# Pixie8888/R3DFSSeg

Measured on AMD Instinct MI355X. Metric: episodes/sec S3DIS 2-way 5-shot 2048-pt (MPTI+attention, train step: forward+backward+grad all-reduce+Adam), higher is better.
Workload: dtype f32 (index-free GEMMs -- self-attention, 1x1 convolutions, weight gradients, the EdgeConv backward's edge GEMMs -- as bf16x3 split products on the bf16 MFMA with fp32 accumulate; every index-deciding result: fp32)

## Files before the change

### include/r3d.h

```cpp
#ifndef R3D_H
#define R3D_H
#include <stdint.h>

#ifdef __cplusplus
extern "C" {
#endif

const char* r3d_last_error_string(void);
int r3d_abi_version(void);
int r3d_debug_poison_lds(unsigned pattern, unsigned* sink , void* stream);
int r3d_debug_set_cg_spmv_lds_min_blocks(int min_blocks);
int r3d_set_matrix_arith(int mode);
int r3d_get_matrix_arith(void);
int r3d_debug_set_gemm_bx3(int mask);

int r3d_cm_to_pm(const float* in , int B, int C, int N, float* out , long ld, void* stream);
int r3d_pm_to_cm(const float* in , long ld, int B, int C, int N, float* out , void* stream);
long r3d_cm_pitch(int N);
int r3d_copy_cols(const float* src, long ld_src, float* dst, long ld_dst, long M, int C, void* stream);

long r3d_knn_norm_ws_words(int B, int N);
int r3d_knn_topk(const float* x, long ldx, const float* x_cm, int B, int N, int C, int k, int mode,
                 const int32_t* n_valid_dev, float* norm_ws, float* cm_ws, int32_t* idx_out, float* score_out,
                 int32_t* status, void* stream);
// ... 46 lines not shown
                        int max_iter, float tol, float* Z, int32_t* ws, long ws_words, int32_t* stats_out, void* stream);

int r3d_label_propagate_batched(int n_ep, const float* nodes, long ldn, int D, const int32_t* nbr, int kp1, const float* Y,
                                const int32_t* n_dev, const int32_t* n_proto_dev, long desc_stride, int n_cap, float sigma,
                                float alpha, int max_iter, float tol, float* Z, int32_t* ws, long ws_words, long ws_stride,
                                int32_t* stats_out, long stats_stride, void* stream);
long r3d_graph_weights_verify_words(int n_cap, int kp1);
int r3d_graph_weights_verify(int n_ep, const float* nodes, long ldn, int D, const int32_t* n_dev, long desc_stride, int n_cap,
                             int kp1, float sigma, int32_t* ws, long ws_words, long ws_stride, float* scratch,
                             int32_t* mismatch_out, void* stream);

int r3d_label_propagate_solve_batched(int n_ep, const float* Y, const int32_t* n_dev, long desc_stride, int n_cap, int kp1,
                                      float alpha, int max_iter, float tol, float* Z, int32_t* ws, long ws_words,
                                      long ws_stride, int32_t* stats_out, long stats_stride, void* stream);

int r3d_graph_set_lp_budget(void* graph, void* graph_exec, int budget, int* n_cg);

int r3d_query_logits_ce_batched(int n_ep, const float* Z, long z_ep_rows, const int32_t* n_proto_dev, long desc_stride, int n_q,
                                int N, int n_classes, const int64_t* labels, float* logits, float* loss_out, int32_t* pred_out,
                                void* stream);

int r3d_pointwise_conv_acc(const float* X, long ldx, const float* W, long M, int K, int Co, const float* scale,
                           const float* shift, int act, float* Out, long ldo, void* stream);
long r3d_pointwise_conv_stats_ws_words(long M, int Co);
int r3d_pointwise_conv_stats(const float* X, long ldx, const float* W, long M, int K, int Co, float* Out, long ldo,
                             float* sums_out , float* ws, void* stream);
int r3d_pointwise_conv_stats_seg(const float* X, long ldx, const float* W, long M, int K, int Co, float* Out, long ldo,
                                 long rows_a, long rows_b, float* sums_out, float* ws, void* stream);
long r3d_colstats_seg_ws_words(long M, int C, long rows_a, long rows_b);
int r3d_colstats_seg(const float* X, long ldx, const float* DY, long lddy, long M, int C, long rows_a, long rows_b, int mode,
                     const float* scale, const float* shift, const float* mean, const float* invstd, long bn_stride, int act,
                     float* sums_out , float* ws, void* stream);
int r3d_bn_fold_seg(const float* sums , int n_seg, double count_a, double count_b, int C, const float* gamma,
                    const float* beta, float eps, float momentum, float* running_mean , float* running_var ,
                    float* mean, float* invstd, float* scale, float* shift, long bn_stride, float* rec ,
                    const int32_t* rec_index_dev , long rec_stride, void* stream);
int r3d_affine_act_seg(const float* Z, long ldz, long M, int C, long rows_a, long rows_b, const float* scale, const float* shift,
                       long bn_stride, int act, float* Y, long ldy, void* stream);
int r3d_bn_bwd_apply_seg(const float* Z, long ldz, const float* DY, long lddy, long M, int C, long rows_a, long rows_b,
                         const float* scale, const float* shift, const float* mean, const float* invstd, long bn_stride, int act,
                         const float* sums , double count_a, double count_b, float* DZ, long lddz, void* stream);
int r3d_bn_running_update(const float* rec, int n_records, long rec_stride, int C, float momentum,
                          const float* bias , float* running_mean,
                          float* running_var, void* stream);
long r3d_gemm_tn_ws_words(long M, int Ca, int Cb);
int r3d_gemm_tn(const float* A, long lda, const float* B, long ldb, long M, int Ca, int Cb, float alpha, float* out,
                int accumulate, float* ws, void* stream);
int r3d_add_cols(const float* src, long ld_src, float* dst, long ld_dst, long M, int C, void* stream);

long r3d_edgeconv_train_ws_words(int B, int N);
int r3d_edge_stats1(const float* PQ, const int32_t* idx, int B, int N, int K, int clouds_a, int clouds_b,
                    float* sums_out , float* esum , float* ws,
                    void* stream);
int r3d_edgeconv_train_fwd_minmax(const float* PQ, const int32_t* idx, const float* s1, const float* t1, long bn_stride,
                                  const float* W2, int B, int N, int K, int clouds_a, int clouds_b, float* zmax, float* zmin,
                                  int32_t* argmax, int32_t* argmin, float* sums_out , float* ws, void* stream);
int r3d_edge_select(float* zmax , const float* zmin, int32_t* argmax ,
                    const int32_t* argmin, const float* s2, const float* t2, long bn_stride, long M, long rows_a, long rows_b,
                    float* out, long ldo, void* stream);
long r3d_edge_reverse_ws_words(int B, int N, int K);
int r3d_edge_reverse(const int32_t* idx, int B, int N, int K, int32_t* rev_ws, long ws_words, void* stream);
int r3d_edgeconv_bwd(const float* PQ, const int32_t* idx, const float* s1, const float* t1, const float* mean1,
                     const float* invstd1, const float* W2, const float* s2, const float* t2, const float* mean2,
                     const float* invstd2, long bn_stride, const float* bn2_sums, const float* dout, long lddo,
                     const int32_t* argmax, const float* zwin , const float* esum , int B, int N, int K,
                     int clouds_a, int clouds_b, float* DY1 , float* BE ,
                     const int32_t* rev_ws , float* dW2, float* bn1_sums, float* dPQ,
                     float* ws, void* stream);

int r3d_ce_grad_batched(int n_ep, const float* Z, const int32_t* n_proto_dev, long desc_stride, int n_cap, int n_query_pts,
                        int n_classes, const int64_t* labels, const float* gscale_dev, float* G, void* stream);
int r3d_label_propagate_bwd_batched(int n_ep, const float* nodes, long ldn, int D, int kp1, const float* Z, const float* G,
                                    const int32_t* n_dev, long desc_stride, int n_cap, float sigma, float alpha, int max_iter,
                                    float tol, float* lam, float* dnodes, long ldd, int32_t* ws, long ws_words, long ws_stride,
                                    int32_t* stats_out, long stats_stride, void* stream);
int r3d_head_prototypes_bwd_batched(int n_ep, const float* dnodes, long ldd, long nodes_ep_rows, int n_way, int k_shot, int N,
                                    int D, int n_query_pts, const int32_t* desc, long desc_stride, const int32_t* assign,
                                    long assign_stride, const int32_t* cluster_count, long ccount_stride, const int32_t* ws,
                                    long ws_stride, float* dsfeat, long lds_, long dsfeat_ep_rows, float* dqfeat, long ldq,
                                    long dqfeat_ep_rows, void* stream);

long r3d_contrast_ws_words(int n_way, int k_shot, int N);
int r3d_contrast_fwd(const float* feat, long ldf, int D, const int32_t* support_y, const int32_t* support_flag, int n_way,
                     int k_shot, int N, const float* W, const float* bias, float temp, float* loss_out, float* ws,
                     long ws_words, void* stream);
int r3d_contrast_bwd(int D, int n_way, int k_shot, int N, const float* gscale_dev, float* dfeat, long ldd, float* dW,
                     float* db, float* ws, void* stream);
int r3d_contrast_fwd_batched(int n_ep, const float* feat, long ldf, long feat_ep_rows, int D, const int32_t* support_y,
                             const int32_t* support_flag, int n_way, int k_shot, int N, const float* W, const float* bias,
                             float temp, float* loss_out, float* ws, long ws_words, long ws_stride, void* stream);
int r3d_contrast_bwd_batched(int n_ep, int D, int n_way, int k_shot, int N, const float* gscale_dev, float* dfeat, long ldd,
                             long dfeat_ep_rows, float* dW, float* db, float* ws, long ws_stride, void* stream);
int r3d_train_metrics_batched(int n_ep, const int32_t* pred, const int64_t* query_y, const int64_t* gt_query_y, int n_query_pts,
                              const float* Z, long z_ep_rows, const int32_t* desc, long desc_stride, const int32_t* proto_ws,
                              long pws_stride, const int32_t* assign, long assign_stride, const int32_t* gt_support_y, int n_way,
                              int k_shot, int N, float* out4 , void* stream);

long r3d_clean_ws_words(int n_way, int k_shot);
int r3d_clean_shot_detect_batched(int n_ep, const float* feat, long ldf, long feat_ep_rows, int D, const float* support_x,
                                  int Cin, const int32_t* support_y, int n_way, int k_shot, int N, int32_t* shot_keep,
                                  float* dbg_cos_sum, int32_t* ws, long ws_stride, void* stream);

int r3d_protonet_head(const float* sfeat, long ldf, const float* qfeat, long ldq, int D, const int32_t* support_y,
                      int n_way, int k_shot, int N, int n_query_pts, int method, float scaler, float* Z, float* ws,
                      void* stream);

long r3d_protonet_head_ws_words(int n_ep, int n_way, int k_shot);
int r3d_protonet_head_batched(int n_ep, const float* sfeat, long ldf, const float* qfeat, long ldq, long feat_ep_rows, int D,
                              const int32_t* support_y, int n_way, int k_shot, int N, int n_query_pts, int method,
                              float scaler, float* Z, float* ws, long ws_words, void* stream);
int r3d_count_correct_batched(int n_ep, const int32_t* pred, const int64_t* labels, long n_pts, int32_t* correct,
                              void* stream);
// ... 22 lines not shown
```

### r3dfsseg_amd/csrc/edgeconv_train.hip

```cpp
#include <stdlib.h>
#include "edge_tile.h"

#define ET_LD 65
#define ET_MAXBLK 1024
#define EC_CHUNK 32

static __device__ __forceinline__ float lrelu(float v) { return v > 0.f ? v : 0.2f * v; }

struct EcGeom {
  int N, cpc;
  __host__ __device__ static EcGeom make(int N) { return EcGeom{N, (N + EC_CHUNK - 1) / EC_CHUNK}; }
  __device__ void range(int chunk, int& cloud, int& p0, int& p1) const {
    cloud = __builtin_amdgcn_readfirstlane(chunk / cpc);
    p0 = __builtin_amdgcn_readfirstlane(cloud * N + (chunk - cloud * cpc) * EC_CHUNK);
    p1 = __builtin_amdgcn_readfirstlane(min(p0 + EC_CHUNK, (cloud + 1) * N));
  }
};
static __device__ __forceinline__ int ec_seg(const r3d_segmap& cs, int cloud) {
  return __builtin_amdgcn_readfirstlane(cs.seg_of_row32(cloud));
}

template <int RT>
__global__ __launch_bounds__(256) void r3d_edge_stats1_kernel(const float* __restrict__ PQ, const int* __restrict__ idx,
                                                              EcGeom gm, int n_chunks, float* __restrict__ part,
// ... 180 lines not shown
#pragma unroll 4
      for (int s = 0; s < 4 * RT; ++s) {
        const int e = 16 * (s >> 2) + 4 * g + (s & 3);
        const float a = G[e * E2_LD + 16 * w + n];
        const float4 b = *(const float4*)(H + e * E2_LD + 4 * n);
        dw[0] = mfma16(a, b.x, dw[0]);
        dw[1] = mfma16(a, b.y, dw[1]);
        dw[2] = mfma16(a, b.z, dw[2]);
        dw[3] = mfma16(a, b.w, dw[3]);
      }
      __syncthreads();
#pragma unroll
      for (int t = 0; t < RT; ++t) {
#pragma unroll
        for (int i = 0; i < 4; ++i) G[(16 * t + 4 * g + i) * E2_LD + c] = acc[t][i];
      }
      __syncthreads();
      {
        float* drow = DY1 + ((pt0 + w) * K) * 64 + lane;
        const float* grow = G + (K * w) * E2_LD + lane;
        float bs = 0.f, es = 0.f;
#pragma unroll
        for (int t = 0; t < K; ++t) {
          const float v = grow[t * E2_LD];
          drow[t * 64] = v;
          bs += v;
          es += eh[t];
          sdye += v * eh[t];
        }
        sdy += bs;
        BE[(pt0 + w) * 128 + lane] = bs;
        BE[(pt0 + w) * 128 + 64 + lane] = es;
      }
    }
    float (*ps)[2][64] = (float (*)[2][64])dsm;
    ps[w][0][lane] = sdy;
    ps[w][1][lane] = sdye;
    __syncthreads();
    if (tid < 128) {
      const int v = tid >> 6, cc = tid & 63;
      part_bn[((long)chunk * 2 + v) * 64 + cc] = ((ps[0][v][cc] + ps[1][v][cc]) + ps[2][v][cc]) + ps[3][v][cc];
    }
    __syncthreads();
  }
  int tid2 = threadIdx.x;
  asm volatile("" : "+v"(tid2));
  const int w2 = tid2 >> 6, n2 = tid2 & 15, g2 = (tid2 >> 4) & 3;
  float* mypart = part_dw + (long)blockIdx.x * 4096;
#pragma unroll
  for (int i = 0; i < 4; ++i)
    *(float4*)(mypart + (16 * w2 + 4 * g2 + i) * 64 + 4 * n2) = float4{dw[0][i], dw[1][i], dw[2][i], dw[3][i]};
}

template <int RT>
__global__ __launch_bounds__(256) void r3d_edgeconv_train_fwd2_kernel(
    const float* __restrict__ PQ, const int* __restrict__ idx, const float* __restrict__ s1, const float* __restrict__ t1,
    long bn_stride, const float* __restrict__ W2, EcGeom gm, r3d_segmap cs , int n_chunks,
    int* __restrict__ argmax_out, float* __restrict__ zmax_out, float* __restrict__ zmin_out, int* __restrict__ argmin_out,
    float* __restrict__ part ) {
  constexpr int K = 4 * RT, R = 16 * RT;
  extern __shared__ __attribute__((aligned(16))) float smem[];
  float* H = smem;
  float* Z = smem + R * E2_LD;
  const int tid = threadIdx.x, lane = tid & 63, w = tid >> 6;
  const int n = lane & 15, g = lane >> 4;
  const int c = 16 * w + n;
  const int N = gm.N;
  float Bz[16];
#pragma unroll
  for (int s = 0; s < 16; ++s) Bz[s] = W2[c * 64 + 16 * g + s];
  for (int item = blockIdx.x; item < n_chunks; item += gridDim.x) {
    const int chunk = r3d_xcd_swizzle(item, n_chunks);
    int cloud, p0, p1;
    gm.range(chunk, cloud, p0, p1);
    const long cloud0 = (long)cloud * N;
    const long bo = (long)ec_seg(cs, cloud) * bn_stride;
    const float sc1 = s1[bo + lane], sh1 = t1[bo + lane];
    float za = 0.f, zb = 0.f;
    for (int pt0_ = p0; pt0_ < p1; pt0_ += E2_PTS) {
      const long pt0 = pt0_;
      {
        const int my_idx = min(max(idx[(pt0 + w) * K + min(lane, K - 1)], 0), N - 1);
        const float q = PQ[(pt0 + w) * 128 + 64 + lane];
        float pv[K];
#pragma unroll
        for (int t = 0; t < K; ++t) pv[t] = PQ[(cloud0 + __builtin_amdgcn_readlane(my_idx, t)) * 128 + lane];
        float* hrow = H + (K * w) * E2_LD + lane;
#pragma unroll
        for (int t = 0; t < K; ++t) hrow[t * E2_LD] = lrelu(sc1 * (pv[t] + q) + sh1);
      }
      __syncthreads();
      f32x4 acc[RT];
      e2_rowgemm<RT>(H, Bz, n, g, acc);
#pragma unroll
      for (int t = 0; t < RT; ++t) {
#pragma unroll
        for (int i = 0; i < 4; ++i) {
          const float z = acc[t][i];
          za += z;
          zb += z * z;
          Z[(16 * t + 4 * g + i) * E2_LD + c] = z;
        }
      }
      __syncthreads();
      {
        const float* zp = Z + (K * w) * E2_LD + lane;
        float zx = zp[0], zn = zx;
        int ax = 0, an = 0;
#pragma unroll
        for (int t = 1; t < K; ++t) {
          const float z = zp[t * E2_LD];
          if (z > zx) { zx = z; ax = t; }
          if (z < zn) { zn = z; an = t; }
        }
        const long o = (pt0 + w) * 64 + lane;
        zmax_out[o] = zx;
        zmin_out[o] = zn;
        argmax_out[o] = ax;
        argmin_out[o] = an;
      }
    }
    za += __shfl_xor(za, 16); zb += __shfl_xor(zb, 16);
    za += __shfl_xor(za, 32); zb += __shfl_xor(zb, 32);
    if (g == 0) {
      part[((long)chunk * 2 + 0) * 64 + c] = za;
      part[((long)chunk * 2 + 1) * 64 + c] = zb;
    }
  }
}

#define RV_RANGE 256
#define RV_CAP 12288
__global__ __launch_bounds__(1024) void r3d_edge_reverse_kernel(const int* __restrict__ idx, int N, int K, int n_clouds,
                                                                int* __restrict__ rev_ptr, int* __restrict__ rev) {
  __shared__ int cnt[RV_RANGE];
  __shared__ int off[RV_RANGE + 1];
  __shared__ int cur[RV_RANGE];
  __shared__ int buf[RV_CAP];
  __shared__ int wsum[16];
  __shared__ int below_s, b_s;
  const int tid = threadIdx.x, lane = tid & 63, w = tid >> 6;
  const int cloud = blockIdx.y;
  const int r0 = blockIdx.x * RV_RANGE, nr = min(RV_RANGE, N - r0);
  const long E = (long)N * K, gbase = (long)cloud * E;
  const int* lst = idx + gbase;
  if (tid < RV_RANGE) cnt[tid] = 0;
  if (tid == 0) below_s = 0;
  __syncthreads();
  int my_below = 0;
  for (long e0 = tid; e0 < E; e0 += 8 * 1024) {
    int jv[8];
#pragma unroll
    for (int u = 0; u < 8; ++u) jv[u] = lst[min(e0 + 1024 * u, E - 1)];
#pragma unroll
    for (int u = 0; u < 8; ++u) {
      const int j = min(max(jv[u], 0), N - 1) - r0;
      if (e0 + 1024 * u < E) {
        if (j < 0) ++my_below;
        else if (j < nr) atomicAdd(&cnt[j], 1);
      }
    }
  }
#pragma unroll
  for (int o = 32; o > 0; o >>= 1) my_below += __shfl_xor(my_below, o);
  if (lane == 0) atomicAdd(&below_s, my_below);
  __syncthreads();
  if (tid < RV_RANGE) {
    const int v = tid < nr ? cnt[tid] : 0;
    int x = v;
#pragma unroll
    for (int o = 1; o < 64; o <<= 1) {
      const int y = __shfl_up(x, o);
      if (lane >= o) x += y;
    }
    if (lane == 63) wsum[w] = x;
    cur[tid] = x - v;
  }
  __syncthreads();
  if (tid < RV_RANGE) {
    int wb = 0;
    for (int q = 0; q < w; ++q) wb += wsum[q];
// ... 189 lines not shown
    }
  }
}

static int et_check(const char* fn, int B, int N, int K, int clouds_a, int clouds_b) {
  if (B <= 0 || N <= 0 || N % E2_PTS != 0 || K < 4 || K > 32 || K % 4 != 0) {
    r3d_set_error("%s: unsupported shape B=%d N=%d K=%d (N %% 4 == 0, K %% 4 == 0, 4..32)", fn, B, N, K);
    return R3D_ERR_ARG;
  }
  const r3d_segmap cs{clouds_a, clouds_b};
  if (!cs.covers(B)) {
    r3d_set_error("%s: %d clouds are not whole segments of %d + %d clouds", fn, B, clouds_a, clouds_b);
    return R3D_ERR_ARG;
  }
  if ((long)B * N * K >= 0x7fffffffL) {
    r3d_set_error("%s: B*N*K = %ld edges exceed the 31-bit edge ids", fn, (long)B * N * K);
    return R3D_ERR_ARG;
  }
  return 0;
}
static int et_chunks(int B, int N) { return B * EcGeom::make(N).cpc; }
static int et_grid8(int n_chunks, int cap) { return n_chunks <= cap ? n_chunks : (cap >= 8 ? cap & ~7 : cap); }

extern "C" long r3d_edgeconv_train_ws_words(int B, int N) { return (long)ET_MAXBLK * 4096 + (long)et_chunks(B, N) * 128 + 64; }

static void et_reduce_chunks(const float* part, int N, int clouds_a, int clouds_b, int n_seg, float* out, hipStream_t st) {
  const int cpc = EcGeom::make(N).cpc;
  hipLaunchKernelGGL(r3d_part_reduce_kernel, dim3(128 / 64, n_seg), dim3(1024), 0, st, part, clouds_a * cpc, clouds_b * cpc, 128,
                     out, 128L, 128, (float*)nullptr, 0L);
}

extern "C" int r3d_edge_stats1(const float* PQ, const int32_t* idx, int B, int N, int K, int clouds_a, int clouds_b,
                               float* sums_out, float* esum, float* ws, void* stream) {
  R3D_REQUIRE(PQ && idx && sums_out && ws, "r3d_edge_stats1: null pointer");
  int rc = et_check("r3d_edge_stats1", B, N, K, clouds_a, clouds_b);
  if (rc) return rc;
  hipStream_t st = (hipStream_t)stream;
  const EcGeom gm = EcGeom::make(N);
  const int n_chunks = et_chunks(B, N);
  const int grid = et_grid8(n_chunks, 2048);
#define E2_CASE(RT) \
  case RT: hipLaunchKernelGGL(r3d_edge_stats1_kernel<RT>, dim3(grid), dim3(256), 0, st, PQ, idx, gm, n_chunks, ws, esum); break
  switch (K / 4) {
    E2_CASE(1); E2_CASE(2); E2_CASE(3); E2_CASE(4); E2_CASE(5); E2_CASE(6); E2_CASE(7); E2_CASE(8);
  }
#undef E2_CASE
  et_reduce_chunks(ws, N, clouds_a, clouds_b, r3d_segmap{clouds_a, clouds_b}.n_seg(B), sums_out, st);
  R3D_LAUNCH_CHECK("r3d_edge_stats1");
  return R3D_OK;
}

template <int RT>
static int fwd2_launch_rt(int n_chunks, hipStream_t st, const float* PQ, const int32_t* idx, const float* s1, const float* t1,
                          long bn_stride, const float* W2, EcGeom gm, r3d_segmap cs, int32_t* argmax, float* zmax, float* zmin,
                          int32_t* argmin, float* ws) {
  const size_t lds = sizeof(float) * ((size_t)2 * 16 * RT * E2_LD);
  static int resident = 0;
  if (!resident) {
    resident = e2_resident_blocks(r3d_edgeconv_train_fwd2_kernel<RT>, lds, ET_MAXBLK);
    R3D_REQUIRE(resident > 0, "r3d_edgeconv_train_fwd_minmax: cannot reserve %zu B of LDS", lds);
  }
  const int grid = et_grid8(n_chunks, resident);
  hipLaunchKernelGGL(r3d_edgeconv_train_fwd2_kernel<RT>, dim3(grid), dim3(256), lds, st, PQ, idx, s1, t1, bn_stride, W2, gm, cs,
                     n_chunks, argmax, zmax, zmin, argmin, ws);
  return R3D_OK;
}

extern "C" int r3d_edgeconv_train_fwd_minmax(const float* PQ, const int32_t* idx, const float* s1, const float* t1,
                                             long bn_stride, const float* W2, int B, int N, int K, int clouds_a, int clouds_b,
                                             float* zmax, float* zmin, int32_t* argmax, int32_t* argmin, float* sums_out,
                                             float* ws, void* stream) {
  R3D_REQUIRE(PQ && idx && s1 && t1 && W2 && zmax && zmin && argmax && argmin && sums_out && ws,
              "r3d_edgeconv_train_fwd_minmax: null pointer");
  int rc = et_check("r3d_edgeconv_train_fwd_minmax", B, N, K, clouds_a, clouds_b);
  if (rc) return rc;
  hipStream_t st = (hipStream_t)stream;
  const EcGeom gm = EcGeom::make(N);
  const r3d_segmap cs{clouds_a, clouds_b};
  const int n_chunks = et_chunks(B, N);
#define E2_CASE(RT)                                                                                                    \
  case RT:                                                                                                             \
    rc = fwd2_launch_rt<RT>(n_chunks, st, PQ, idx, s1, t1, bn_stride, W2, gm, cs, argmax, zmax, zmin, argmin, ws);      \
    break
  switch (K / 4) {
    E2_CASE(1); E2_CASE(2); E2_CASE(3); E2_CASE(4); E2_CASE(5); E2_CASE(6); E2_CASE(7); E2_CASE(8);
  }
#undef E2_CASE
  if (rc) return rc;
  et_reduce_chunks(ws, N, clouds_a, clouds_b, cs.n_seg(B), sums_out, st);
  R3D_LAUNCH_CHECK("r3d_edgeconv_train_fwd_minmax");
  return R3D_OK;
}

__global__ void r3d_edge_select_kernel(float* __restrict__ zmax, const float* __restrict__ zmin, int* __restrict__ argmax,
                                       const int* __restrict__ argmin, const float* __restrict__ s2,
                                       const float* __restrict__ t2, long bn_stride, r3d_segmap sm , long M,
                                       float* __restrict__ out, long ldo) {
  const long i = (long)blockIdx.x * blockDim.x + threadIdx.x;
  if (i >= M * 64) return;
  const int c = (int)(i & 63);
  const long m = (long)__builtin_amdgcn_readfirstlane((int)(i >> 6));
  const long bo = (long)__builtin_amdgcn_readfirstlane(sm.seg_of_row32((int)m)) * bn_stride + c;
  const float sc = s2[bo];
  const bool up = sc >= 0.f;
  const float z = up ? zmax[i] : zmin[i];
  if (!up) { zmax[i] = z; argmax[i] = argmin[i]; }
  out[m * ldo + c] = lrelu(sc * z + t2[bo]);
}
extern "C" int r3d_edge_select(float* zmax, const float* zmin, int32_t* argmax, const int32_t* argmin, const float* s2,
                               const float* t2, long bn_stride, long M, long rows_a, long rows_b, float* out, long ldo,
                               void* stream) {
  R3D_REQUIRE(zmax && zmin && argmax && argmin && s2 && t2 && out && M > 0 && ldo >= 64, "r3d_edge_select: bad arguments");
  const r3d_segmap sm{rows_a, rows_b};
  R3D_REQUIRE(sm.covers(M), "r3d_edge_select: %ld rows are not whole segments of %ld + %ld rows", M, rows_a, rows_b);
  hipLaunchKernelGGL(r3d_edge_select_kernel, dim3(r3d_cdiv(M * 64, 256)), dim3(256), 0, (hipStream_t)stream, zmax, zmin,
                     argmax, argmin, s2, t2, bn_stride, sm, M, out, ldo);
  R3D_LAUNCH_CHECK("r3d_edge_select");
  return R3D_OK;
}

template <int RT>
static int bwd1_launch_rt(int n_chunks, hipStream_t st, const float* PQ, const int32_t* idx, EcBn bn, const float* W2,
                          const float* bn2_sums, const float* dout, long lddo, const int32_t* argmax, EcGeom gm, r3d_segmap cs,
                          float* DY1, float* BE, float* part_dw, float* part_bn, int* grid_out) {
  const size_t lds = sizeof(float) * ((size_t)2 * 16 * RT * E2_LD + 2 * E2_PTS * 64 + 6 * 64);
  static int resident = 0;
  if (!resident) {
    resident = e2_resident_blocks(r3d_edgeconv_bwd1_kernel<RT>, lds, ET_MAXBLK);
    R3D_REQUIRE(resident > 0, "r3d_edgeconv_bwd: cannot reserve %zu B of LDS", lds);
  }
  const int grid = et_grid8(n_chunks, resident);
  hipLaunchKernelGGL(r3d_edgeconv_bwd1_kernel<RT>, dim3(grid), dim3(256), lds, st, PQ, idx, bn, W2, bn2_sums, dout, lddo, argmax,
                     gm, cs, n_chunks, DY1, BE, part_dw, part_bn);
  *grid_out = grid;
  return R3D_OK;
}

template <int RT>
static int bwd1_bx3_launch_rt(int n_chunks, hipStream_t st, const float* PQ, const int32_t* idx, EcBn bn, const float* W2,
                              const float* bn2_sums, const float* dout, long lddo, const int32_t* argmax, const float* zwin,
                              EcGeom gm, r3d_segmap cs, float* DY1, float* BE, float* part_dw, float* part_bn, int* grid_out) {
  static int resident = 0;
  if (!resident) {
    resident = e2_resident_blocks(r3d_edgeconv_bwd1_bx3_kernel<RT>, EB_LDS_BYTES, ET_MAXBLK / 2);
    R3D_REQUIRE(resident > 0, "r3d_edgeconv_bwd: cannot reserve %d B of LDS", (int)EB_LDS_BYTES);
  }
  const int grid = et_grid8(n_chunks, resident);
  hipLaunchKernelGGL(r3d_edgeconv_bwd1_bx3_kernel<RT>, dim3(grid), dim3(256), EB_LDS_BYTES, st, PQ, idx, bn, W2, bn2_sums, dout,
                     lddo, argmax, zwin, gm, cs, n_chunks, DY1, BE, part_dw, part_bn);
  *grid_out = grid;
  return R3D_OK;
}

extern "C" long r3d_edge_reverse_ws_words(int B, int N, int K) { return (long)B * N + 1 + (long)B * N * K + 16; }
extern "C" int r3d_edge_reverse(const int32_t* idx, int B, int N, int K, int32_t* rev_ws, long ws_words, void* stream) {
  R3D_REQUIRE(idx && rev_ws, "r3d_edge_reverse: null pointer");
  R3D_REQUIRE(B > 0 && B <= 65535 && N > 0 && K > 0 && (long)B * N * K < 0x7fffffffL, "r3d_edge_reverse: bad shape B=%d N=%d K=%d",
              B, N, K);
  R3D_REQUIRE(ws_words >= r3d_edge_reverse_ws_words(B, N, K), "r3d_edge_reverse: workspace of %ld words is shorter than "
              "r3d_edge_reverse_ws_words(%d, %d, %d)", ws_words, B, N, K);
  const size_t ro_lds = sizeof(int) * (size_t)RO_WAVES * N;
  static const bool ro_off = getenv("R3D_EDGE_REVERSE_SORT") != nullptr;
  if (!ro_off && ro_lds <= 144 * 1024 && (long)N * K >= 64 * RO_WAVES) {
    static size_t attr = 0;
    if (ro_lds > attr) {
      R3D_REQUIRE(hipFuncSetAttribute((const void*)r3d_edge_reverse_ordered_kernel, hipFuncAttributeMaxDynamicSharedMemorySize,
                                      (int)ro_lds) == hipSuccess, "r3d_edge_reverse: cannot reserve %zu B of LDS", ro_lds);
      attr = ro_lds;
    }
    hipLaunchKernelGGL(r3d_edge_reverse_ordered_kernel, dim3(B), dim3(64 * RO_WAVES), ro_lds, (hipStream_t)stream, idx, N, K, B,
// ... 61 lines not shown
```

### r3dfsseg_amd/train_ops.py

```python
import contextlib
import ctypes
from collections import namedtuple

import torch

from . import _lib, ops
from .ops import SegLayout, _p, _rows, _st, _timed

BN_EPS, BN_MOM = 1e-5, 0.1
update_running_stats = True


class BNRecorder:

    def __init__(self, max_episodes, device):
        self.max_records = 2 * max_episodes
        self.device = device
        self.tables = {}
        self.index_dev = None

    def slot_for(self, bnmod, bias):
        if bnmod not in self.tables:
            rec = torch.zeros(self.max_records, 2, bnmod.num_features, device=self.device, dtype=torch.float32)
            self.tables[bnmod] = (rec, bias.detach() if bias is not None else None)
# ... 144 lines not shown
    M, ldx = _rows(X)
    C = W2d.shape[0]
    lib = _lib.load()
    seg = _one_segment(M) if seg is None else seg
    assert seg.M == M
    z = torch.empty(M, C, device=X.device, dtype=torch.float32)
    if seg.aligned(64):
        sums = _f(seg.n_seg * 2 * C, X.device).view(seg.n_seg, 2, C)
        ws = _f(lib.r3d_pointwise_conv_stats_ws_words(M, C), X.device)
        with _timed("pointwise_conv"):
            _lib.check(lib.r3d_pointwise_conv_stats_seg(_p(X), ldx, _p(W2d), M, X.shape[1], C, _p(z), C, seg.rows_a, seg.rows_b,
                                                        _p(sums), _p(ws), _st()))
    else:
        ops.pointwise_conv(X, W2d, out=z)
        sums = colstats(z, C, seg, mode=0)
    bn = bn_fold(sums, seg.counts(), bnmod, bias)
    y = affine_act(z, bn, act, seg, out=out)
    return y, (X, W2d, z, bn, act, seg)


def conv_bn_bwd(saved, dY, want_dx=True, dx_acc=None):
    X, W2d, z, bn, act, seg = saved
    C = W2d.shape[0]
    M = z.shape[0]
    sums = colstats(z, C, seg, mode=1, DY=dY, bn=bn, act=act)
    dz = bn_bwd_apply(z, dY, bn, act, sums, seg.counts(), seg)
    dW = gemm_tn(dz, X)
    tot = sums.sum(0) if seg.n_seg > 1 else sums[0]
    dbias = torch.zeros(C, device=z.device, dtype=torch.float32)
    dX = None
    if want_dx:
        Wt = W2d.t().contiguous()
        if dx_acc is not None:
            conv_acc(dz, Wt, dx_acc)
        else:
            dX = ops.pointwise_conv(dz, Wt)
    return dW, tot[1], tot[0], dbias, dX


def edgeconv_train_fwd(inp, idx, ec, B, N, out, seg=None):
    lib = _lib.load()
    dev = inp.device
    seg = SegLayout(1, B, 0, N) if seg is None else seg
    assert seg.B == B and seg.N == N
    W1 = ec.layer[0].weight.reshape(64, -1)
    C = W1.shape[1] // 2
    Wpq = torch.cat((W1[:, :C], W1[:, C:] - W1[:, :C]), 0).contiguous()
    PQ = ops.pointwise_conv(inp, Wpq)
    K = idx.shape[-1]
    ws = _f(lib.r3d_edgeconv_train_ws_words(B, N), dev)
    W2 = ec.layer[3].weight.reshape(64, 64).contiguous()
    M = B * N
    argmax = torch.empty(M, 64, device=dev, dtype=torch.int32)
    argmin = torch.empty(M, 64, device=dev, dtype=torch.int32)
    zmax = torch.empty(M, 64, device=dev, dtype=torch.float32)
    zmin = torch.empty(M, 64, device=dev, dtype=torch.float32)
    idx3 = idx.view(B, N, K)
    sums1 = _f(seg.n_seg * 128, dev).view(seg.n_seg, 2, 64)
    sums2 = _f(seg.n_seg * 128, dev).view(seg.n_seg, 2, 64)
    counts = seg.counts(per_row=K)
    esum = torch.empty(M, 64, device=dev, dtype=torch.float32)
    with _timed("edgeconv"):
        _lib.check(lib.r3d_edge_stats1(_p(PQ), _p(idx3), B, N, K, seg.S, seg.Q, _p(sums1), _p(esum), _p(ws), _st()))
    bn1 = bn_fold(sums1, counts, ec.layer[1])
    sc1, sh1, _, _ = bn1.ptrs()
    with _timed("edgeconv"):
        _lib.check(lib.r3d_edgeconv_train_fwd_minmax(_p(PQ), _p(idx3), sc1, sh1, bn1.stride, _p(W2), B, N, K, seg.S, seg.Q,
                                                     _p(zmax), _p(zmin), _p(argmax), _p(argmin), _p(sums2), _p(ws), _st()))
    bn2 = bn_fold(sums2, counts, ec.layer[4])
    sc2, sh2, _, _ = bn2.ptrs()
    with _timed("edgeconv"):
        _lib.check(lib.r3d_edge_select(_p(zmax), _p(zmin), _p(argmax), _p(argmin), sc2, sh2, bn2.stride, M, seg.rows_a,
                                       seg.rows_b, _p(out), out.stride(0), _st()))
    return (inp, idx3, Wpq, PQ, W2, bn1, bn2, argmax, zmax, C, seg, esum)


def edgeconv_train_bwd(saved, dout, B, N, dx_acc):
    inp, idx3, Wpq, PQ, W2, bn1, bn2, argmax, zmax, C, seg, esum = saved
    lib = _lib.load()
    dev = PQ.device
    K = idx3.shape[-1]
    M = B * N
    dPQ = _f(M * 128, dev).view(M, 128)
    ws = _f(lib.r3d_edgeconv_train_ws_words(B, N), dev)
    rev = torch.empty(lib.r3d_edge_reverse_ws_words(B, N, K), device=dev, dtype=torch.int32)
    with _timed("edgeconv_bwd"):
        _lib.check(lib.r3d_edge_reverse(_p(idx3), B, N, K, _p(rev), rev.numel(), _st()))
    bn2_sums = colstats(zmax, 64, seg, mode=1, DY=dout, bn=bn2, act=ops.ACT_LRELU)
    DY1, BE = _f(M * K * 64, dev), _f(M * 128, dev)
    dW2, bn1_sums = _f(64 * 64, dev), _f(seg.n_seg * 128, dev).view(seg.n_seg, 2, 64)
    s1, t1, m1, i1 = bn1.ptrs()
    s2, t2, m2, i2 = bn2.ptrs()
    with _timed("edgeconv_bwd"):
        _lib.check(lib.r3d_edgeconv_bwd(_p(PQ), _p(idx3), s1, t1, m1, i1, _p(W2), s2, t2, m2, i2, bn1.stride, _p(bn2_sums),
                                        _p(dout), dout.stride(0), _p(argmax), _p(zmax), _p(esum), B, N, K, seg.S, seg.Q, _p(DY1),
                                        _p(BE), _p(rev),
                                        _p(dW2), _p(bn1_sums), _p(dPQ), _p(ws), _st()))
    t1s = bn1_sums.sum(0) if seg.n_seg > 1 else bn1_sums[0]
    t2s = bn2_sums.sum(0) if seg.n_seg > 1 else bn2_sums[0]
    dWpq = gemm_tn(dPQ, inp)
    dW1 = torch.cat((dWpq[:64] - dWpq[64:], dWpq[64:]), 1).reshape(64, 2 * C, 1, 1)
    if dx_acc is not None:
        conv_acc(dPQ, Wpq.t().contiguous(), dx_acc)
    return dW1, t1s[1], t1s[0], dW2.view(64, 64, 1, 1), t2s[1], t2s[0]


EncoderSaved = namedtuple("EncoderSaved", "model seg seed p_drop seed_dev ec mlp base cat level2 qkv lse feat aws")


def encoder_forward(model, x, seed, seg=None):
    enc, base, att = model.encoder, model.base_learner, model.att_learner
    lib = _lib.load()
    B, _, N = x.shape
    M = B * N
    dev = x.device
    if seg is None:
        seg = SegLayout(1, B, 0, N)
    assert seg.B == B and seg.N == N
    x_pm, x_cm = ops.input_layouts(x)
    cat = torch.empty(M, 64 * enc.n_edgeconv, device=dev, dtype=torch.float32)
    inp, ec_saved = x_pm, []
    for l in range(enc.n_edgeconv):
        idx = ops.knn(inp, B, N, enc.k, x_cm=x_cm if l == 0 else None)
        if enc.idx_patch is not None:
            idx = enc.idx_patch(l, idx.view(B, N, enc.k)).view(idx.shape)
        out = cat[:, 64 * l:64 * (l + 1)]
        ec_saved.append(edgeconv_train_fwd(inp, idx, enc.edge_convs[l], B, N, out, seg))
        inp = out
    h, mlp_saved = cat, []
    for jn in range(len(enc.conv.layer_dims)):
        W = enc.conv.layer[3 * jn].weight
        h, sv = conv_bn_fwd(h, W.reshape(W.shape[0], -1).contiguous(), enc.conv.layer[3 * jn + 1], ops.ACT_LRELU, seg=seg)
        mlp_saved.append(sv)
    level2 = h
    feat = torch.empty(M, model.feat_dim, device=dev, dtype=torch.float32)
    od = att.out_channel
    ops.copy_cols(cat[:, :64], feat[:, :64])
    hb, base_saved = level2, []
    for i, seq in enumerate(base.convs):
        last = i == base.num_convs - 1
        W = seq[0].weight
        hb, sv = conv_bn_fwd(hb, W.reshape(W.shape[0], -1).contiguous(), seq[1], ops.ACT_NONE if last else ops.ACT_RELU,
                             bias=seq[0].bias, out=feat[:, 64 + od:] if last else None, seg=seg)
        base_saved.append(sv)
    Wqkv, qscale = att._fold()
    qkv = ops.pointwise_conv(level2, Wqkv, qscale, None, ops.ACT_NONE)
    lse = torch.empty(M, device=dev, dtype=torch.float32)
    p_drop = float(att.dropout.p)
# ... 150 lines not shown
```

Baseline: 384.9.

## Select EdgeConv max/min winner in-register using BN gamma sign, double-buffer gather

The EdgeConv forward kernel now reads the sign of BN2's gamma to decide whether each channel keeps the max or the min over neighbours. It picks that winner directly from the MFMA accumulators with a sign-flip trick and permlane swaps, writing only one value and one index instead of max, min and both argmax/argmin. This drops the Z staging in LDS, one barrier per tile, half the output writes and the separate edge_select kernel, which is replaced by a generic affine_act. The gather of the next tile's neighbour features and indices is software-pipelined through cursors and double-buffered H in LDS. The risks are more register pressure and a dependence on gamma's sign standing in for the folded BN scale's sign, which holds if the folded scale is gamma times a positive inverse std.

Result: no change. 388.5, median of 6 (+1.0%).

```diff
diff --git a/include/r3d.h b/include/r3d.h
--- a/include/r3d.h
+++ b/include/r3d.h
@@ -122,12 +122,9 @@
 int r3d_edge_stats1(const float* PQ, const int32_t* idx, int B, int N, int K, int clouds_a, int clouds_b,
                     float* sums_out , float* esum , float* ws,
                     void* stream);
-int r3d_edgeconv_train_fwd_minmax(const float* PQ, const int32_t* idx, const float* s1, const float* t1, long bn_stride,
-                                  const float* W2, int B, int N, int K, int clouds_a, int clouds_b, float* zmax, float* zmin,
-                                  int32_t* argmax, int32_t* argmin, float* sums_out , float* ws, void* stream);
-int r3d_edge_select(float* zmax , const float* zmin, int32_t* argmax ,
-                    const int32_t* argmin, const float* s2, const float* t2, long bn_stride, long M, long rows_a, long rows_b,
-                    float* out, long ldo, void* stream);
+int r3d_edgeconv_train_fwd_win(const float* PQ, const int32_t* idx, const float* s1, const float* t1, long bn_stride,
+                               const float* W2, const float* gamma2, int B, int N, int K, int clouds_a, int clouds_b,
+                               float* zwin, int32_t* argwin, float* sums_out , float* ws, void* stream);
 long r3d_edge_reverse_ws_words(int B, int N, int K);
 int r3d_edge_reverse(const int32_t* idx, int B, int N, int K, int32_t* rev_ws, long ws_words, void* stream);
 int r3d_edgeconv_bwd(const float* PQ, const int32_t* idx, const float* s1, const float* t1, const float* mean1,
diff --git a/r3dfsseg_amd/csrc/edgeconv_train.hip b/r3dfsseg_amd/csrc/edgeconv_train.hip
--- a/r3dfsseg_amd/csrc/edgeconv_train.hip
+++ b/r3dfsseg_amd/csrc/edgeconv_train.hip
@@ -256,81 +256,149 @@
     *(float4*)(mypart + (16 * w2 + 4 * g2 + i) * 64 + 4 * n2) = float4{dw[0][i], dw[1][i], dw[2][i], dw[3][i]};
 }
 
+struct EcCursor {
+  int item, chunk, cloud, p0, p1, pt0;
+  long bo;
+  __device__ bool valid(int n_chunks) const { return item < n_chunks; }
+  __device__ void open(const EcGeom& gm, const r3d_segmap& cs, long bn_stride, int n_chunks) {
+    if (item < n_chunks) {
+      chunk = r3d_xcd_swizzle(item, n_chunks);
+      gm.range(chunk, cloud, p0, p1);
+      pt0 = p0;
+      bo = (long)ec_seg(cs, cloud) * bn_stride;
+    }
+  }
+  __device__ void next(const EcGeom& gm, const r3d_segmap& cs, long bn_stride, int n_chunks, int stride) {
+    pt0 += E2_PTS;
+    if (pt0 >= p1 && item < n_chunks) {
+      item += stride;
+      open(gm, cs, bn_stride, n_chunks);
+    }
+  }
+};
+
+static __device__ __forceinline__ void ec_better(float& av, int& ap, float bv, int bp) {
+  const bool take = (bv > av) | ((bv == av) & (bp < ap));
+  av = take ? bv : av;
+  ap = take ? bp : ap;
+}
+
 template <int RT>
 __global__ __launch_bounds__(256) void r3d_edgeconv_train_fwd2_kernel(
     const float* __restrict__ PQ, const int* __restrict__ idx, const float* __restrict__ s1, const float* __restrict__ t1,
-    long bn_stride, const float* __restrict__ W2, EcGeom gm, r3d_segmap cs , int n_chunks,
-    int* __restrict__ argmax_out, float* __restrict__ zmax_out, float* __restrict__ zmin_out, int* __restrict__ argmin_out,
-    float* __restrict__ part ) {
+    long bn_stride, const float* __restrict__ W2, const float* __restrict__ gamma2, EcGeom gm, r3d_segmap cs ,
+    int n_chunks, int* __restrict__ argwin_out, float* __restrict__ zwin_out, float* __restrict__ part ) {
   constexpr int K = 4 * RT, R = 16 * RT;
   extern __shared__ __attribute__((aligned(16))) float smem[];
-  float* H = smem;
-  float* Z = smem + R * E2_LD;
   const int tid = threadIdx.x, lane = tid & 63, w = tid >> 6;
   const int n = lane & 15, g = lane >> 4;
   const int c = 16 * w + n;
   const int N = gm.N;
+  const int stride = gridDim.x;
   float Bz[16];
 #pragma unroll
   for (int s = 0; s < 16; ++s) Bz[s] = W2[c * 64 + 16 * g + s];
-  for (int item = blockIdx.x; item < n_chunks; item += gridDim.x) {
-    const int chunk = r3d_xcd_swizzle(item, n_chunks);
-    int cloud, p0, p1;
-    gm.range(chunk, cloud, p0, p1);
-    const long cloud0 = (long)cloud * N;
-    const long bo = (long)ec_seg(cs, cloud) * bn_stride;
-    const float sc1 = s1[bo + lane], sh1 = t1[bo + lane];
-    float za = 0.f, zb = 0.f;
-    for (int pt0_ = p0; pt0_ < p1; pt0_ += E2_PTS) {
-      const long pt0 = pt0_;
-      {
-        const int my_idx = min(max(idx[(pt0 + w) * K + min(lane, K - 1)], 0), N - 1);
-        const float q = PQ[(pt0 + w) * 128 + 64 + lane];
-        float pv[K];
-#pragma unroll
-        for (int t = 0; t < K; ++t) pv[t] = PQ[(cloud0 + __builtin_amdgcn_readlane(my_idx, t)) * 128 + lane];
-        float* hrow = H + (K * w) * E2_LD + lane;
-#pragma unroll
-        for (int t = 0; t < K; ++t) hrow[t * E2_LD] = lrelu(sc1 * (pv[t] + q) + sh1);
-      }
-      __syncthreads();
-      f32x4 acc[RT];
-      e2_rowgemm<RT>(H, Bz, n, g, acc);
-#pragma unroll
-      for (int t = 0; t < RT; ++t) {
-#pragma unroll
-        for (int i = 0; i < 4; ++i) {
-          const float z = acc[t][i];
-          za += z;
-          zb += z * z;
-          Z[(16 * t + 4 * g + i) * E2_LD + c] = z;
+  const unsigned flip = !(gamma2[c] >= 0.f) ? 0x80000000u : 0u;
+  EcCursor cu{(int)blockIdx.x, 0, 0, 0, 0, 0, 0};
+  cu.open(gm, cs, bn_stride, n_chunks);
+  if (!cu.valid(n_chunks)) return;
+  EcCursor c1 = cu, c2 = cu;
+  float pv[K], q, sc1, sh1;
+  int nidx;
+#define EC_LOAD_IDX(cur) nidx = idx[(long)((cur).pt0 + w) * K + min(lane, K - 1)]
+#define EC_GATHER(cur)                                                                                                       \
+  {                                                                                                                          \
+    const int my_idx = min(max(nidx, 0), N - 1);                \
+    const long cloud0 = (long)(cur).cloud * N;                                                                               \
+    q = PQ[(long)((cur).pt0 + w) * 128 + 64 + lane];                                                                         \
+    _Pragma("unroll") for (int t = 0; t < K; ++t) pv[t] = PQ[(cloud0 + __builtin_amdgcn_readlane(my_idx, t)) * 128 + lane]; \
+    sc1 = s1[(cur).bo + lane];                                                                                               \
+    sh1 = t1[(cur).bo + lane];                                                                                               \
+  }
+  EC_LOAD_IDX(c1);
+  EC_GATHER(c1);
+  c1.next(gm, cs, bn_stride, n_chunks, stride);
+  c2.next(gm, cs, bn_stride, n_chunks, stride);
+  if (c1.valid(n_chunks)) EC_LOAD_IDX(c1);
+  c2.next(gm, cs, bn_stride, n_chunks, stride);
+  float za = 0.f, zb = 0.f;
+  int buf = 0;
+  while (true) {
+    {
+      float* hrow = smem + buf * (R * E2_LD) + (K * w) * E2_LD + lane;
+#pragma unroll
+      for (int t = 0; t < K; ++t) hrow[t * E2_LD] = lrelu(sc1 * (pv[t] + q) + sh1);
+    }
+    if (c1.valid(n_chunks)) EC_GATHER(c1);
+    if (c2.valid(n_chunks)) EC_LOAD_IDX(c2);
+    __syncthreads();
+    f32x4 acc[RT];
+    e2_rowgemm<RT>(smem + buf * (R * E2_LD), Bz, n, g, acc);
+    float bv[E2_PTS];
+    int bp[E2_PTS];
+#pragma unroll
+    for (int p = 0; p < E2_PTS; ++p) { bv[p] = -__builtin_inff(); bp[p] = K; }
+#pragma unroll
+    for (int t = 0; t < RT; ++t) {
+      float v = 0.f;
+      int vi = 0;
+#pragma unroll
+      for (int i = 0; i < 4; ++i) {
+        const float z = acc[t][i];
+        za += z;
+        zb += z * z;
+        const float y = __uint_as_float(__float_as_uint(z) ^ flip);
+        if (i == 0 || y > v) { v = y; vi = i; }
+      }
+      const int e0 = 16 * t + 4 * g;
+#pragma unroll
+      for (int p = 0; p < E2_PTS; ++p) {
+        if (p * K < 16 * t + 16 && (p + 1) * K > 16 * t) {
+          const bool mine = e0 >= p * K && e0 < (p + 1) * K;
+          const bool take = mine && v > bv[p];
+          bv[p] = take ? v : bv[p];
+          bp[p] = take ? e0 - p * K + vi : bp[p];
         }
       }
-      __syncthreads();
-      {
-        const float* zp = Z + (K * w) * E2_LD + lane;
-        float zx = zp[0], zn = zx;
-        int ax = 0, an = 0;
-#pragma unroll
-        for (int t = 1; t < K; ++t) {
-          const float z = zp[t * E2_LD];
-          if (z > zx) { zx = z; ax = t; }
-          if (z < zn) { zn = z; an = t; }
-        }
-        const long o = (pt0 + w) * 64 + lane;
-        zmax_out[o] = zx;
-        zmin_out[o] = zn;
-        argmax_out[o] = ax;
-        argmin_out[o] = an;
-      }
-    }
-    za += __shfl_xor(za, 16); zb += __shfl_xor(zb, 16);
-    za += __shfl_xor(za, 32); zb += __shfl_xor(zb, 32);
-    if (g == 0) {
-      part[((long)chunk * 2 + 0) * 64 + c] = za;
-      part[((long)chunk * 2 + 1) * 64 + c] = zb;
-    }
-  }
+    }
+    float rv[2];
+    int rp[2];
+#pragma unroll
+    for (int j = 0; j < 2; ++j) {
+      const auto sv = __builtin_amdgcn_permlane32_swap(__float_as_uint(bv[j]), __float_as_uint(bv[2 + j]), false, false);
+      const auto sp = __builtin_amdgcn_permlane32_swap((unsigned)bp[j], (unsigned)bp[2 + j], false, false);
+      rv[j] = __uint_as_float(sv[0]);
+      rp[j] = (int)sp[0];
+      ec_better(rv[j], rp[j], __uint_as_float(sv[1]), (int)sp[1]);
+    }
+    {
+      const auto sv = __builtin_amdgcn_permlane16_swap(__float_as_uint(rv[0]), __float_as_uint(rv[1]), false, false);
+      const auto sp = __builtin_amdgcn_permlane16_swap((unsigned)rp[0], (unsigned)rp[1], false, false);
+      float fv = __uint_as_float(sv[0]);
+      int fp = (int)sp[0];
+      ec_better(fv, fp, __uint_as_float(sv[1]), (int)sp[1]);
+      const long o = (long)(cu.pt0 + g) * 64 + c;
+      zwin_out[o] = __uint_as_float(__float_as_uint(fv) ^ flip);
+      argwin_out[o] = fp < K ? fp : 0;
+    }
+    if (cu.pt0 + E2_PTS >= cu.p1) {
+      za += __shfl_xor(za, 16); zb += __shfl_xor(zb, 16);
+      za += __shfl_xor(za, 32); zb += __shfl_xor(zb, 32);
+      if (g == 0) {
+        part[((long)cu.chunk * 2 + 0) * 64 + c] = za;
+        part[((long)cu.chunk * 2 + 1) * 64 + c] = zb;
+      }
+      za = 0.f;
+      zb = 0.f;
+    }
+    cu.next(gm, cs, bn_stride, n_chunks, stride);
+    c1.next(gm, cs, bn_stride, n_chunks, stride);
+    c2.next(gm, cs, bn_stride, n_chunks, stride);
+    if (!cu.valid(n_chunks)) break;
+    buf ^= 1;
+  }
+#undef EC_LOAD_IDX
+#undef EC_GATHER
 }
 
 #define RV_RANGE 256
@@ -626,27 +694,26 @@
 
 template <int RT>
 static int fwd2_launch_rt(int n_chunks, hipStream_t st, const float* PQ, const int32_t* idx, const float* s1, const float* t1,
-                          long bn_stride, const float* W2, EcGeom gm, r3d_segmap cs, int32_t* argmax, float* zmax, float* zmin,
-                          int32_t* argmin, float* ws) {
+                          long bn_stride, const float* W2, const float* gamma2, EcGeom gm, r3d_segmap cs, int32_t* argwin,
+                          float* zwin, float* ws) {
   const size_t lds = sizeof(float) * ((size_t)2 * 16 * RT * E2_LD);
   static int resident = 0;
   if (!resident) {
     resident = e2_resident_blocks(r3d_edgeconv_train_fwd2_kernel<RT>, lds, ET_MAXBLK);
-    R3D_REQUIRE(resident > 0, "r3d_edgeconv_train_fwd_minmax: cannot reserve %zu B of LDS", lds);
+    R3D_REQUIRE(resident > 0, "r3d_edgeconv_train_fwd_win: cannot reserve %zu B of LDS", lds);
   }
   const int grid = et_grid8(n_chunks, resident);
-  hipLaunchKernelGGL(r3d_edgeconv_train_fwd2_kernel<RT>, dim3(grid), dim3(256), lds, st, PQ, idx, s1, t1, bn_stride, W2, gm, cs,
-                     n_chunks, argmax, zmax, zmin, argmin, ws);
+  hipLaunchKernelGGL(r3d_edgeconv_train_fwd2_kernel<RT>, dim3(grid), dim3(256), lds, st, PQ, idx, s1, t1, bn_stride, W2, gamma2,
+                     gm, cs, n_chunks, argwin, zwin, ws);
   return R3D_OK;
 }
 
-extern "C" int r3d_edgeconv_train_fwd_minmax(const float* PQ, const int32_t* idx, const float* s1, const float* t1,
-                                             long bn_stride, const float* W2, int B, int N, int K, int clouds_a, int clouds_b,
-                                             float* zmax, float* zmin, int32_t* argmax, int32_t* argmin, float* sums_out,
-                                             float* ws, void* stream) {
-  R3D_REQUIRE(PQ && idx && s1 && t1 && W2 && zmax && zmin && argmax && argmin && sums_out && ws,
-              "r3d_edgeconv_train_fwd_minmax: null pointer");
-  int rc = et_check("r3d_edgeconv_train_fwd_minmax", B, N, K, clouds_a, clouds_b);
+extern "C" int r3d_edgeconv_train_fwd_win(const float* PQ, const int32_t* idx, const float* s1, const float* t1, long bn_stride,
+                                          const float* W2, const float* gamma2, int B, int N, int K, int clouds_a, int clouds_b,
+                                          float* zwin, int32_t* argwin, float* sums_out, float* ws, void* stream) {
+  R3D_REQUIRE(PQ && idx && s1 && t1 && W2 && gamma2 && zwin && argwin && sums_out && ws,
+              "r3d_edgeconv_train_fwd_win: null pointer");
+  int rc = et_check("r3d_edgeconv_train_fwd_win", B, N, K, clouds_a, clouds_b);
   if (rc) return rc;
   hipStream_t st = (hipStream_t)stream;
   const EcGeom gm = EcGeom::make(N);
@@ -654,7 +721,7 @@
   const int n_chunks = et_chunks(B, N);
 #define E2_CASE(RT)                                                                                                    \
   case RT:                                                                                                             \
-    rc = fwd2_launch_rt<RT>(n_chunks, st, PQ, idx, s1, t1, bn_stride, W2, gm, cs, argmax, zmax, zmin, argmin, ws);      \
+    rc = fwd2_launch_rt<RT>(n_chunks, st, PQ, idx, s1, t1, bn_stride, W2, gamma2, gm, cs, argwin, zwin, ws);           \
     break
   switch (K / 4) {
     E2_CASE(1); E2_CASE(2); E2_CASE(3); E2_CASE(4); E2_CASE(5); E2_CASE(6); E2_CASE(7); E2_CASE(8);
@@ -662,34 +729,7 @@
 #undef E2_CASE
   if (rc) return rc;
   et_reduce_chunks(ws, N, clouds_a, clouds_b, cs.n_seg(B), sums_out, st);
-  R3D_LAUNCH_CHECK("r3d_edgeconv_train_fwd_minmax");
-  return R3D_OK;
-}
-
-__global__ void r3d_edge_select_kernel(float* __restrict__ zmax, const float* __restrict__ zmin, int* __restrict__ argmax,
-                                       const int* __restrict__ argmin, const float* __restrict__ s2,
-                                       const float* __restrict__ t2, long bn_stride, r3d_segmap sm , long M,
-                                       float* __restrict__ out, long ldo) {
-  const long i = (long)blockIdx.x * blockDim.x + threadIdx.x;
-  if (i >= M * 64) return;
-  const int c = (int)(i & 63);
-  const long m = (long)__builtin_amdgcn_readfirstlane((int)(i >> 6));
-  const long bo = (long)__builtin_amdgcn_readfirstlane(sm.seg_of_row32((int)m)) * bn_stride + c;
-  const float sc = s2[bo];
-  const bool up = sc >= 0.f;
-  const float z = up ? zmax[i] : zmin[i];
-  if (!up) { zmax[i] = z; argmax[i] = argmin[i]; }
-  out[m * ldo + c] = lrelu(sc * z + t2[bo]);
-}
-extern "C" int r3d_edge_select(float* zmax, const float* zmin, int32_t* argmax, const int32_t* argmin, const float* s2,
-                               const float* t2, long bn_stride, long M, long rows_a, long rows_b, float* out, long ldo,
-                               void* stream) {
-  R3D_REQUIRE(zmax && zmin && argmax && argmin && s2 && t2 && out && M > 0 && ldo >= 64, "r3d_edge_select: bad arguments");
-  const r3d_segmap sm{rows_a, rows_b};
-  R3D_REQUIRE(sm.covers(M), "r3d_edge_select: %ld rows are not whole segments of %ld + %ld rows", M, rows_a, rows_b);
-  hipLaunchKernelGGL(r3d_edge_select_kernel, dim3(r3d_cdiv(M * 64, 256)), dim3(256), 0, (hipStream_t)stream, zmax, zmin,
-                     argmax, argmin, s2, t2, bn_stride, sm, M, out, ldo);
-  R3D_LAUNCH_CHECK("r3d_edge_select");
+  R3D_LAUNCH_CHECK("r3d_edgeconv_train_fwd_win");
   return R3D_OK;
 }
 
diff --git a/r3dfsseg_amd/train_ops.py b/r3dfsseg_amd/train_ops.py
--- a/r3dfsseg_amd/train_ops.py
+++ b/r3dfsseg_amd/train_ops.py
@@ -220,9 +220,7 @@
     W2 = ec.layer[3].weight.reshape(64, 64).contiguous()
     M = B * N
     argmax = torch.empty(M, 64, device=dev, dtype=torch.int32)
-    argmin = torch.empty(M, 64, device=dev, dtype=torch.int32)
-    zmax = torch.empty(M, 64, device=dev, dtype=torch.float32)
-    zmin = torch.empty(M, 64, device=dev, dtype=torch.float32)
+    zwin = torch.empty(M, 64, device=dev, dtype=torch.float32)
     idx3 = idx.view(B, N, K)
     sums1 = _f(seg.n_seg * 128, dev).view(seg.n_seg, 2, 64)
     sums2 = _f(seg.n_seg * 128, dev).view(seg.n_seg, 2, 64)
@@ -232,19 +230,18 @@
         _lib.check(lib.r3d_edge_stats1(_p(PQ), _p(idx3), B, N, K, seg.S, seg.Q, _p(sums1), _p(esum), _p(ws), _st()))
     bn1 = bn_fold(sums1, counts, ec.layer[1])
     sc1, sh1, _, _ = bn1.ptrs()
+    gamma2 = ec.layer[4].weight.detach().contiguous()
     with _timed("edgeconv"):
-        _lib.check(lib.r3d_edgeconv_train_fwd_minmax(_p(PQ), _p(idx3), sc1, sh1, bn1.stride, _p(W2), B, N, K, seg.S, seg.Q,
-                                                     _p(zmax), _p(zmin), _p(argmax), _p(argmin), _p(sums2), _p(ws), _st()))
+        _lib.check(lib.r3d_edgeconv_train_fwd_win(_p(PQ), _p(idx3), sc1, sh1, bn1.stride, _p(W2), _p(gamma2), B, N, K, seg.S,
+                                                  seg.Q, _p(zwin), _p(argmax), _p(sums2), _p(ws), _st()))
     bn2 = bn_fold(sums2, counts, ec.layer[4])
-    sc2, sh2, _, _ = bn2.ptrs()
     with _timed("edgeconv"):
-        _lib.check(lib.r3d_edge_select(_p(zmax), _p(zmin), _p(argmax), _p(argmin), sc2, sh2, bn2.stride, M, seg.rows_a,
-                                       seg.rows_b, _p(out), out.stride(0), _st()))
-    return (inp, idx3, Wpq, PQ, W2, bn1, bn2, argmax, zmax, C, seg, esum)
+        affine_act(zwin, bn2, ops.ACT_LRELU, seg, out=out)
+    return (inp, idx3, Wpq, PQ, W2, bn1, bn2, argmax, zwin, C, seg, esum)
 
 
 def edgeconv_train_bwd(saved, dout, B, N, dx_acc):
-    inp, idx3, Wpq, PQ, W2, bn1, bn2, argmax, zmax, C, seg, esum = saved
+    inp, idx3, Wpq, PQ, W2, bn1, bn2, argmax, zwin, C, seg, esum = saved
     lib = _lib.load()
     dev = PQ.device
     K = idx3.shape[-1]
@@ -254,14 +251,14 @@
     rev = torch.empty(lib.r3d_edge_reverse_ws_words(B, N, K), device=dev, dtype=torch.int32)
     with _timed("edgeconv_bwd"):
         _lib.check(lib.r3d_edge_reverse(_p(idx3), B, N, K, _p(rev), rev.numel(), _st()))
-    bn2_sums = colstats(zmax, 64, seg, mode=1, DY=dout, bn=bn2, act=ops.ACT_LRELU)
+    bn2_sums = colstats(zwin, 64, seg, mode=1, DY=dout, bn=bn2, act=ops.ACT_LRELU)
     DY1, BE = _f(M * K * 64, dev), _f(M * 128, dev)
     dW2, bn1_sums = _f(64 * 64, dev), _f(seg.n_seg * 128, dev).view(seg.n_seg, 2, 64)
     s1, t1, m1, i1 = bn1.ptrs()
     s2, t2, m2, i2 = bn2.ptrs()
     with _timed("edgeconv_bwd"):
         _lib.check(lib.r3d_edgeconv_bwd(_p(PQ), _p(idx3), s1, t1, m1, i1, _p(W2), s2, t2, m2, i2, bn1.stride, _p(bn2_sums),
-                                        _p(dout), dout.stride(0), _p(argmax), _p(zmax), _p(esum), B, N, K, seg.S, seg.Q, _p(DY1),
+                                        _p(dout), dout.stride(0), _p(argmax), _p(zwin), _p(esum), B, N, K, seg.S, seg.Q, _p(DY1),
                                         _p(BE), _p(rev),
                                         _p(dW2), _p(bn1_sums), _p(dPQ), _p(ws), _st()))
     t1s = bn1_sums.sum(0) if seg.n_seg > 1 else bn1_sums[0]
```
